# lzhangbj/deep_video_interpolation_extrapolation

Hardware: AMD Instinct MI355X
Metric: train frames/s (256x512 len-3 clips) (higher is better)
Workload: dtype bf16; 1 GPU; InterNet int_5_len_3 train step 256x512 bf16; per_gpu_batch=8, global_batch=8, parallelism=dp1, step=eager, executor side-stream lanes

## Files before the change

deep_video_interpolation_extrapolation_amd/csrc/ew.hip:

```cpp
#include <stdlib.h>

#include "common.h"

namespace dvie {

struct Lerp {
  int i0, i1;
  float l0, l1;
};
__device__ __forceinline__ Lerp lerp_src(int dst, int in_size, int out_size, int align) {
  float src;
  if (align) {
    const float scale = out_size > 1 ? (float)(in_size - 1) / (float)(out_size - 1) : 0.f;
    src = scale * (float)dst;
  } else {
    const float scale = (float)in_size / (float)out_size;
    src = scale * ((float)dst + 0.5f) - 0.5f;
  }
  if (src < 0.f) src = 0.f;
  Lerp r;
  r.i0 = (int)src;
  if (r.i0 > in_size - 1) r.i0 = in_size - 1;
  r.i1 = r.i0 + ((r.i0 < in_size - 1) ? 1 : 0);
  r.l1 = src - (float)r.i0;
// ... 333 lines not shown
#pragma unroll
      for (int k = 0; k < VW; ++k) v[k] += t[k];
    }
    if (p.beta) {
      VecN<T, VW>::load(yp, t);
#pragma unroll
      for (int k = 0; k < VW; ++k) v[k] += t[k];
    }
    if (p.act) {
#pragma unroll
      for (int k = 0; k < VW; ++k) v[k] = act_fwd(v[k], p.act, p.alpha);
    }
    if (p.dact) {
      VecN<T, VW>::load((const T*)p.z + pix * p.z_ld + c, t);
#pragma unroll
      for (int k = 0; k < VW; ++k) v[k] *= act_dz(t[k], p.dact, p.alpha);
    }
    VecN<T, VW>::store(yp, v);
  };
  finish(x, v0);
  if (two) finish(x + 1, v1);
}

template <int R>
__global__ __launch_bounds__(256) void ew_fuser_kernel(const dvie_ew_desc p, int cq) {
  const int e = blockIdx.x * 256 + threadIdx.x;
  const int sw = p.sw0, sh = p.sh0;
  if (e >= sw * cq) return;
  const int q = e / cq;
  const int c = (e - q * cq) * 8;
  const int row = blockIdx.y;
  const int n = row / p.h, y = row - (row / p.h) * p.h;
  const bf16_t* s = (const bf16_t*)p.src0;
  const long long ld = p.src_ld0;
  const Lerp ly = lerp_src(y, sh, p.h, 0);
  const long long r0 = ((long long)n * sh + ly.i0) * sw, r1 = ((long long)n * sh + ly.i1) * sw;
  const int qm = q > 0 ? q - 1 : 0, qp = q + 1 < sw ? q + 1 : sw - 1;
  float tm0[8], t00[8], tp0[8], tm1[8], t01[8], tp1[8];
  VecN<bf16_t, 8>::load(s + (r0 + qm) * ld + c, tm0);
  VecN<bf16_t, 8>::load(s + (r0 + q) * ld + c, t00);
  VecN<bf16_t, 8>::load(s + (r0 + qp) * ld + c, tp0);
  VecN<bf16_t, 8>::load(s + (r1 + qm) * ld + c, tm1);
  VecN<bf16_t, 8>::load(s + (r1 + q) * ld + c, t01);
  VecN<bf16_t, 8>::load(s + (r1 + qp) * ld + c, tp1);
#pragma unroll
  for (int r = 0; r < R; ++r) {
    const int x = R * q + r;
    if (x >= p.w) break;
    const Lerp lx = lerp_src(x, sw, p.w, 0);
    const bool lo = lx.i0 < q, hi = lx.i1 > q;
    float v[8];
#pragma unroll
    for (int k = 0; k < 8; ++k) {
      const float a = lo ? tm0[k] : t00[k], b = hi ? tp0[k] : t00[k];
      const float cc = lo ? tm1[k] : t01[k], d = hi ? tp1[k] : t01[k];
      v[k] = 0.f + (ly.l0 * (lx.l0 * a + lx.l1 * b) + ly.l1 * (lx.l0 * cc + lx.l1 * d));
    }
    const long long pix = (long long)row * p.w + x;
    bf16_t* yp = (bf16_t*)p.y + pix * p.y_ld + c;
    float t[8];
    if (p.res) {
      VecN<bf16_t, 8>::load((const bf16_t*)p.res + pix * p.res_ld + c, t);
#pragma unroll
      for (int k = 0; k < 8; ++k) v[k] += t[k];
    }
    if (p.beta) {
      VecN<bf16_t, 8>::load(yp, t);
#pragma unroll
      for (int k = 0; k < 8; ++k) v[k] += t[k];
    }
    if (p.act) {
#pragma unroll
      for (int k = 0; k < 8; ++k) v[k] = act_fwd(v[k], p.act, p.alpha);
    }
    if (p.dact) {
      VecN<bf16_t, 8>::load((const bf16_t*)p.z + pix * p.z_ld + c, t);
#pragma unroll
      for (int k = 0; k < 8; ++k) v[k] *= act_dz(t[k], p.dact, p.alpha);
    }
    VecN<bf16_t, 8>::store(yp, v);
  }
}

template <int R>
__global__ __launch_bounds__(256) void ew_upt22_kernel(const dvie_ew_desc p, int cq) {
  constexpr int NW = 3 * R;
  const int e = blockIdx.x * 256 + threadIdx.x;
  const int wp = (p.w + 1) >> 1, hp = (p.h + 1) >> 1;
  if (e >= wp * cq) return;
  const int xp = e / cq;
  const int c = (e - xp * cq) * 8;
  const int x = 2 * xp;
  const int rowp = blockIdx.y;
  const int n = rowp / hp, y = 2 * (rowp - (rowp / hp) * hp);
  const bool twox = x + 1 < p.w, twoy = y + 1 < p.h;
  const int sh = p.sh0, sw = p.sw0;
  const long long ld = p.src_ld0;
  const int Y0 = R * y - R / 2, X0 = R * x - R / 2;
  float wx0[NW], wx1[NW];
  unsigned xo[NW];
#pragma unroll
  for (int j = 0; j < NW; ++j) {
    const int X = X0 + j;
    const bool in = X >= 0 && X < sw;
    wx0[j] = in ? upt_weight(X, x, p.w, sw, 0) : 0.f;
    wx1[j] = (in && twox) ? upt_weight(X, x + 1, p.w, sw, 0) : 0.f;
    xo[j] = (unsigned)((in ? X : 0) * ld + c) * 2u;
  }
  const __amdgpu_buffer_rsrc_t rs = __builtin_amdgcn_make_buffer_rsrc((void*)p.src0, 0, 0x7FFFFFF0, 0x00020000);
  float acc[2][2][8];
#pragma unroll
  for (int a = 0; a < 2; ++a)
#pragma unroll
    for (int b = 0; b < 2; ++b)
#pragma unroll
      for (int k = 0; k < 8; ++k) acc[a][b][k] = 0.f;
#pragma unroll 1
  for (int i = 0; i < NW; ++i) {
    const int Y = Y0 + i;
    if (Y < 0 || Y >= sh) continue;
    const float wy0 = upt_weight(Y, y, p.h, sh, 0), wy1 = twoy ? upt_weight(Y, y + 1, p.h, sh, 0) : 0.f;
    if (wy0 == 0.f && wy1 == 0.f) continue;
    const unsigned rowo = (unsigned)(((long long)n * sh + Y) * sw * ld) * 2u;
    i32x4 raw[NW];
#pragma unroll
    for (int j = 0; j < NW; ++j) raw[j] = __builtin_bit_cast(i32x4, __builtin_amdgcn_raw_buffer_load_b128(rs, rowo + xo[j], 0, 0));
    float h0[8], h1[8];
#pragma unroll
    for (int k = 0; k < 8; ++k) h0[k] = h1[k] = 0.f;
#pragma unroll
    for (int j = 0; j < NW; ++j)
#pragma unroll
      for (int k = 0; k < 4; ++k) {
        const float lo = __uint_as_float(((uint32_t)raw[j][k]) << 16), hi = __uint_as_float(((uint32_t)raw[j][k]) & 0xffff0000u);
        h0[2 * k] += wx0[j] * lo;
        h0[2 * k + 1] += wx0[j] * hi;
        h1[2 * k] += wx1[j] * lo;
        h1[2 * k + 1] += wx1[j] * hi;
      }
#pragma unroll
    for (int k = 0; k < 8; ++k) {
      acc[0][0][k] += wy0 * h0[k];
      acc[0][1][k] += wy0 * h1[k];
      acc[1][0][k] += wy1 * h0[k];
      acc[1][1][k] += wy1 * h1[k];
    }
  }
  auto finish = [&](int yy, int xx, float* v) {
    const long long pix = ((long long)n * p.h + yy) * p.w + xx;
    bf16_t* yp = (bf16_t*)p.y + pix * p.y_ld + c;
    float t[8];
    if (p.res) {
      VecN<bf16_t, 8>::load((const bf16_t*)p.res + pix * p.res_ld + c, t);
#pragma unroll
      for (int k = 0; k < 8; ++k) v[k] += t[k];
    }
    if (p.beta) {
      VecN<bf16_t, 8>::load(yp, t);
#pragma unroll
      for (int k = 0; k < 8; ++k) v[k] += t[k];
    }
    if (p.act) {
#pragma unroll
      for (int k = 0; k < 8; ++k) v[k] = act_fwd(v[k], p.act, p.alpha);
    }
    if (p.dact) {
      VecN<bf16_t, 8>::load((const bf16_t*)p.z + pix * p.z_ld + c, t);
#pragma unroll
      for (int k = 0; k < 8; ++k) v[k] *= act_dz(t[k], p.dact, p.alpha);
    }
    VecN<bf16_t, 8>::store(yp, v);
  };
  finish(y, x, acc[0][0]);
  if (twox) finish(y, x + 1, acc[0][1]);
  if (twoy) {
    finish(y + 1, x, acc[1][0]);
    if (twox) finish(y + 1, x + 1, acc[1][1]);
  }
}

__global__ __launch_bounds__(256) void ew_nchw_kernel(const dvie_ew_desc p) {
  const int x = blockIdx.x * 256 + threadIdx.x;
  if (x >= p.w) return;
  const int row = blockIdx.y;
  const int n = row / p.h, y = row - (row / p.h) * p.h;
  const long long pix = (long long)row * p.w + x;
  const long long base = (long long)n * p.sn + (long long)y * p.sh + (long long)x * p.sw;
  if (p.c <= 32) {
    float v[32];
#pragma unroll
    for (int ch = 0; ch < 32; ++ch) {
      float t = 0.f;
      if (ch < p.c && ch < p.ext_c) {
        const bool second = p.src1 != nullptr && ch >= p.sh1;
        const float* e = second ? (const float*)p.src1 : p.ext;
        const int cc = second ? ch - p.sh1 : ch;
        t = e[base + (long long)cc * p.sc];
        if (p.mean) t = (t - p.mean[ch]) / p.std[ch];
      }
      v[ch] = t;
    }
#pragma unroll
    for (int c = 0; c < 32; c += 8)
      if (c < p.c) VecN<bf16_t, 8>::store((bf16_t*)p.y + pix * p.y_ld + c, v + c);
    return;
  }
  for (int c = 0; c < p.c; c += 8) {
    float v[8];
#pragma unroll
    for (int k = 0; k < 8; ++k) {
      const int ch = c + k;
      float t = 0.f;
      if (ch < p.ext_c) {
        const bool second = p.src1 != nullptr && ch >= p.sh1;
        const float* e = second ? (const float*)p.src1 : p.ext;
        const int cc = second ? ch - p.sh1 : ch;
        t = e[base + (long long)cc * p.sc];
        if (p.mean) t = (t - p.mean[ch]) / p.std[ch];
      }
      v[k] = t;
    }
    VecN<bf16_t, 8>::store((bf16_t*)p.y + pix * p.y_ld + c, v);
  }
}

template <typename T, int VW>
__global__ __launch_bounds__(256) void ew_labels_kernel(const dvie_ew_desc p, int cq) {
  const int e = blockIdx.x * 256 + threadIdx.x;
  if (e >= p.w * cq) return;
  const int x = e / cq;
  const int c = (e - x * cq) * VW;
  const int row = blockIdx.y;
  const int n = row / p.h, y = row - (row / p.h) * p.h;
  const uint8_t* lab = (const uint8_t*)p.ext;
  const int l = lab[(long long)n * p.sn + (long long)y * p.sh + (long long)x * p.sw];
  float v[VW];
#pragma unroll
  for (int k = 0; k < VW; ++k) v[k] = (c + k < p.ext_c && l == c + k) ? 1.f : 0.f;
  VecN<T, VW>::store((T*)p.y + ((long long)row * p.w + x) * p.y_ld + c, v);
}

}

using namespace dvie;

static bool fuse2_on() {
  const char* e = getenv("DVIE_EW_FUSE2");
  return !(e && *e == '0');
}

static int fuser_on() {
  const char* e = getenv("DVIE_EW_FUSER");
  return e && *e ? atoi(e) : 1;
}

extern "C" int dvie_ew(const dvie_ew_desc* d, void* stream) {
  DVIE_CHECK_ARG(d && d->c > 0 && d->c % 4 == 0, "ew: c=%d must be a multiple of 4", d ? d->c : -1);
  DVIE_CHECK_ARG(d->n > 0 && d->h > 0 && d->w > 0, "ew: empty shape");
  DVIE_CHECK_ARG(d->op == DVIE_EW_TONCHW || (d->y && d->y_ld % 4 == 0), "ew: y");
  if (d->op == DVIE_EW_POOL) DVIE_CHECK_ARG(d->sh0 == 2 * d->h && d->sw0 == 2 * d->w, "ew: pool shape");
  if (d->op == DVIE_EW_POOLT) DVIE_CHECK_ARG(d->h == 2 * d->sh0 && d->w == 2 * d->sw0, "ew: poolT shape");
  if (d->op == DVIE_EW_NCHW || d->op == DVIE_EW_TONCHW || d->op == DVIE_EW_MASK || d->op == DVIE_EW_LABELS)
    DVIE_CHECK_ARG(d->ext != nullptr, "ew: ext");
  if (d->op == DVIE_EW_LABELS)
    DVIE_CHECK_ARG(d->ext_c > 0 && d->ext_c <= 256 && !d->res && !d->beta && !d->act && !d->dact,
                   "ew: labels ext_c=%d (1..256), no epilogue operands", d->ext_c);
  if (d->dact) DVIE_CHECK_ARG(d->z != nullptr && d->z_ld % 4 == 0, "ew: z");
  if (d->op == DVIE_EW_IM2COL)
    DVIE_CHECK_ARG(d->ext_c > 0 && d->ext_c % 8 == 0 && d->src0 && d->src_ld0 >= d->ext_c &&
                       d->sh0 > 0 && d->sw0 > 0 && d->sh0 * d->sw0 * d->ext_c <= d->c,
                   "ew: im2col ext_c=%d c=%d taps=%dx%d", d->ext_c, d->c, d->sh0, d->sw0);
  DVIE_CHECK_ARG((long long)d->n * d->h < 65536 && (long long)d->w * d->c < (1LL << 30), "ew: grid too large");
  hipStream_t s = (hipStream_t)stream;
  auto al = [](const void* q, long long ld) { return !q || ((((uintptr_t)q) & 15) == 0 && ld % 8 == 0); };
  const bool v8 = d->dtype == DVIE_BF16 && d->c % 8 == 0 && al(d->y, d->y_ld) && al(d->src0, d->src_ld0) &&
                  al(d->src1, d->src_ld1) && al(d->src2, d->src_ld2) && al(d->res, d->res_ld) && al(d->z, d->z_ld);
  const int vw = v8 ? 8 : 4;
  const int cq = d->c / vw;
  const dim3 grid((unsigned)((d->w * cq + 255) / 256), (unsigned)(d->n * d->h));
  if (d->op == DVIE_EW_LABELS) {
    if (d->dtype == DVIE_BF16 && v8)
      DVIE_LAUNCH((ew_labels_kernel<bf16_t, 8>), grid, dim3(256), 0, s, *d, cq);
    else if (d->dtype == DVIE_BF16)
      DVIE_LAUNCH((ew_labels_kernel<bf16_t, 4>), grid, dim3(256), 0, s, *d, cq);
    else
      DVIE_LAUNCH((ew_labels_kernel<float, 4>), grid, dim3(256), 0, s, *d, cq);
    DVIE_RETURN_LAUNCH();
  }
  if (d->dtype == DVIE_BF16) {
    if (v8) {
      const bool up = d->sw0 <= d->w && d->sh0 <= d->h && (d->nsrc < 2 || (d->sw1 <= d->w && d->sh1 <= d->h)) &&
                      (d->nsrc < 3 || (d->sw2 <= d->w && d->sh2 <= d->h));
      if (d->op == DVIE_EW_NCHW && !d->res && !d->beta && !d->act && !d->dact) {
        const dim3 gn((unsigned)((d->w + 255) / 256), (unsigned)(d->n * d->h));
        DVIE_LAUNCH(ew_nchw_kernel, gn, dim3(256), 0, s, *d);
      } else if (d->op == DVIE_EW_FUSE && d->nsrc == 1 && !d->align && fuser_on() &&
                 ((d->h == 4 * d->sh0 && d->w == 4 * d->sw0) || (fuser_on() > 1 && d->h == 2 * d->sh0 && d->w == 2 * d->sw0))) {
        const dim3 gr((unsigned)((d->sw0 * cq + 255) / 256), (unsigned)(d->n * d->h));
        if (d->w == 4 * d->sw0)
          DVIE_LAUNCH((ew_fuser_kernel<4>), gr, dim3(256), 0, s, *d, cq);
        else
          DVIE_LAUNCH((ew_fuser_kernel<2>), gr, dim3(256), 0, s, *d, cq);
      } else if (d->op == DVIE_EW_FUSE && up && fuse2_on()) {
        const dim3 g2((unsigned)((((d->w + 1) / 2) * cq + 255) / 256), (unsigned)(d->n * d->h));
        DVIE_LAUNCH((ew_fuse2_kernel<bf16_t, 8>), g2, dim3(256), 0, s, *d, cq);
      } else if (d->op == DVIE_EW_FUSE)
        DVIE_LAUNCH((ew_kernel<bf16_t, 8, DVIE_EW_FUSE>), grid, dim3(256), 0, s, *d, cq);
      else if (d->op == DVIE_EW_UPT && !d->align &&
               (unsigned long long)d->n * d->sh0 * d->sw0 * d->src_ld0 * 2ull < 0x7FFFFFF0ull &&
               ((d->sh0 == 2 * d->h && d->sw0 == 2 * d->w) || (d->sh0 == 4 * d->h && d->sw0 == 4 * d->w))) {
        const dim3 g4((unsigned)((((d->w + 1) / 2) * cq + 255) / 256), (unsigned)(d->n * ((d->h + 1) / 2)));
        if (d->sh0 == 4 * d->h)
          DVIE_LAUNCH((ew_upt22_kernel<4>), g4, dim3(256), 0, s, *d, cq);
        else
          DVIE_LAUNCH((ew_upt22_kernel<2>), g4, dim3(256), 0, s, *d, cq);
      } else if (d->op == DVIE_EW_UPT)
        DVIE_LAUNCH((ew_kernel<bf16_t, 8, DVIE_EW_UPT>), grid, dim3(256), 0, s, *d, cq);
      else
        DVIE_LAUNCH((ew_kernel<bf16_t, 8, -2>), grid, dim3(256), 0, s, *d, cq);
    } else {
      DVIE_LAUNCH((ew_kernel<bf16_t, 4, -1>), grid, dim3(256), 0, s, *d, cq);
    }
  } else {
    DVIE_LAUNCH((ew_kernel<float, 4, -1>), grid, dim3(256), 0, s, *d, cq);
  }
  DVIE_RETURN_LAUNCH();
}
```

deep_video_interpolation_extrapolation_amd/engine.py:

```python
import ctypes
import os
from typing import NamedTuple, Optional

import torch

from . import _lib as L

PADC = 8
PROFILE = None
DEBUG_NAN = bool(os.environ.get("DVIE_DEBUG_NAN"))
def _wgrad_lane():
    return os.environ.get("DVIE_WGRAD_LANE", "1") != "0"


OP_HOOK = None


def pack_blocks(d):
    n = L.load().dvie_pack_blocks(ctypes.byref(d))
    assert n > 0, "dvie_pack_blocks: empty pack descriptor"
    return n


def _reduce_meta(name, r):
# ... 559 lines not shown
    size = [rup(max(int(b), 1), ARENA_ALIGN) for b, _, _ in items]
    order = sorted(range(len(items)), key=lambda i: (-size[i], items[i][1], i))
    offsets = [0] * len(items)
    placed = []
    arena = 0
    for i in order:
        _, f, l = items[i]
        busy = sorted((offsets[j], offsets[j] + size[j]) for j in placed if items[j][1] <= l and f <= items[j][2])
        off = 0
        for lo, hi in busy:
            if off + size[i] <= lo:
                break
            off = max(off, hi)
        offsets[i] = off
        placed.append(i)
        arena = max(arena, off + size[i])
    if arena > sum(size):
        offsets, arena = [], 0
        for sz in size:
            offsets.append(arena)
            arena += sz
    return offsets, arena


def arena_layout(g, nf):
    life = forward_lifetimes(g, nf)
    n_sites = max([b for _, b in life.values()] + [0])
    bufs = [b for b in g.buffers if not b.external]
    items = []
    for b in bufs:
        nbytes = nf * b.H * b.W * b.C * elem_size(b.dtype or g.dtype)
        items.append((nbytes,) + life.get(id(b), (0, n_sites)))
    offsets, arena = assign_offsets(items)
    return {id(b): o for b, o in zip(bufs, offsets)}, arena, sum(it[0] for it in items)


class Plan:

    def __init__(self, g, nf, nb, device, backward, alias=False):
        assert not (alias and backward), "alias=True is for forward-only plans (a backward reads every activation)"
        self.g, self.nf, self.nb, self.device, self.alias = g, nf, nb, device, alias
        self.dtype = g.dtype
        self.dt = dv_dtype(g.dtype)
        self.es = elem_size(g.dtype)
        self.vec = 16 // self.es
        self.backward_enabled = backward
        self.keep = []
        self.busy = False
        self.generation = 0
        self.static_weights = False
        self._pack_srcs, self._pack_sig, self._pack_descs = [], None, []
        self.arena, self.arena_bytes, self.unaliased_bytes = None, None, 0
        self.l1_out = self.bn_partial = None
        self.bn_splits = 1
        self._seg_bwd, self._seg_inner = {}, set()
        self.fwd = []
        self.bwd = []
        self.fwd_arr = self.bwd_arr = None
        self.fwd_off = self.n_bwd = 0
        self._l1_fwd = []
        self._l1_bwd = []
        self._cos_fwd = []
        self.cos_ws_blocks = 0
        self.ext_in = {}
        self.ext_out = {}
        self.ext_mask = {}
        self.ext_nchw_out = {}
        self.ext_head = {}
        self.ext_head_grad = {}
        self.keep_grad = None
        self.ext_grad = {}
        self._grad_slots = []
        self.ext_ograd = {}
        self.wg_first = {}
        self._uses_left = {}
        self.completions = []
        self._multi = []
        self._i2c = None
        self.ws = None
        self.ws_floats = 1
        self.zbits = {}
        self._zbits_level = int(os.environ.get("DVIE_ZBITS", "1") or 0)
        self._zbits_on = self._zbits_level > 0
        self._fwd_conv = {}
        self._zb = {}
        self._alloc()
        self._build_pack()
        self._build_forward()
        if backward:
            self._build_backward()
        assert all(o.lane == 0 for o in self.fwd), "forward ops run on the caller's stream"
        self._finalize()

    def _alloc(self):
        g = self.g
        offsets, self.arena_bytes, self.unaliased_bytes = arena_layout(g, self.nf) if self.alias else ({}, None, 0)
        if self.alias:
            self.arena = torch.empty(max(self.arena_bytes, ARENA_ALIGN), dtype=torch.uint8, device=self.device)
            self.keep.append(self.arena)
        for b in g.buffers:
            dt = b.dtype or self.dtype
            b.dt = dt
            if b.external:
                b.t = None
            elif self.alias:
                nbytes = self.nf * b.H * b.W * b.C * elem_size(dt)
                o = offsets[id(b)]
                b.t = self.arena[o:o + nbytes].view(dt).view(self.nf, b.H, b.W, b.C)
            else:
                b.t = torch.empty((self.nf, b.H, b.W, b.C), dtype=dt, device=self.device)
                self.unaliased_bytes += b.t.numel() * b.t.element_size()
        if self.backward_enabled:
            for op in g.ops:
                if op.out is None:
                    continue
                need = False
                if isinstance(op, InputOp):
                    need = op.requires_grad
                elif isinstance(op, (ConvOp, ConvTOp)):
                    need = op.layer.trainable or any(r.buf.needs_grad for r in op.inputs())
                elif isinstance(op, BNOp):
                    need = op.trainable or op.x.buf.needs_grad
                elif isinstance(op, FuseOp) and op.detach:
                    need = False
                else:
                    need = any(r.buf.needs_grad for r in op.inputs())
                op.out.buf.needs_grad = op.out.buf.needs_grad or need
            self._seg_bwd = self._segenc_bwd_chains()
            self._seg_inner = {id(op.out.buf) for ch in self._seg_bwd.values() for op in ch[:2]}
            for b in g.buffers:
                if b.needs_grad and id(b) not in self._seg_inner:
                    b.g = torch.zeros((self.nb, b.H, b.W, b.C), dtype=self.dtype, device=self.device)
            for b in g.buffers:
                b.expected, b.pending = {}, {}
                b.n_flushed = 0
                b.done = b.dact_done = False
            for op in g.ops:
                if isinstance(op, FuseOp) and op.detach:
                    continue
                for r in op.inputs():
                    if r.buf.needs_grad:
                        r.buf.expected[r.key()] = r.buf.expected.get(r.key(), 0) + 1
            for b in g.buffers:
                keys = sorted(b.expected)
                for (a0, ac), (b0, _) in zip(keys, keys[1:]):
                    assert a0 + ac <= b0, f"{b}: consumers read overlapping regions {keys}"
        self.l1_out = torch.zeros(max(1, g.n_l1), dtype=torch.float32, device=self.device)
        self.keep.append(self.l1_out)
        doubles = 8
        for op in g.ops:
            if isinstance(op, BNOp):
                d = L.BnDesc()
                d.c = op.x.c
                for n in (self.nf, self.nb):
                    d.rows = n * op.x.H * op.x.W
                    self.bn_splits = max(self.bn_splits, L.load().dvie_bn_partial_splits(ctypes.byref(d)))
                    doubles = max(doubles, L.load().dvie_bn_partial_doubles(ctypes.byref(d)))
                op.stats = torch.zeros((8, op.x.c), dtype=torch.float32, device=self.device)
                self.keep.append(op.stats)
        self.bn_partial = torch.zeros(doubles, dtype=torch.float64, device=self.device)
        self.keep.append(self.bn_partial)

    def ptr(self, region, n0=0, grad=False):
        b = region.buf
        t = b.g if grad else b.t
        es = elem_size(t.dtype)
# ... 345 lines not shown
        cb = sum(b.c for b in op.bs)
        moved = {"l2norm": 4 * op.c, "softmax": 3 * J, "wnorm": 4 * J, "pool": 2 * op.c,
                 "corr": op.c + J + cb, "gather": out.c + J + cb}[op.kind]

        def contrib(region, build):
            if region.buf.needs_grad:
                def emit(epi):
                    o = build(epi._asdict())
                    o.meta = dict(cls="attn_bwd", name=f"{op.kind}:{region.buf.name}", flops=0.0,
                                  bytes=float(self.es * npx * moved))
                    return [o]
                self._contrib(region, emit)

        if op.kind == "l2norm":
            contrib(a, lambda e: self.attn_desc(L.ATTN_L2NORM_BWD, nb, hw, op.c, gout, gld, self.ptr(a, grad=True),
                                                ld_a, self.ptr(out), self.ptr(a), self._same_ld(out, a), **e))
        elif op.kind == "softmax":
            contrib(a, lambda e: self.attn_desc(L.ATTN_SOFTMAX_BWD, nb, hw, op.c, gout, gld, self.ptr(a, grad=True),
                                                ld_a, self.ptr(out), None, out.buf.C, op.wh, op.ww, op.nhalf, **e))
        elif op.kind == "wnorm":
            contrib(a, lambda e: self.attn_desc(L.ATTN_WNORM_BWD, nb, hw, op.c, gout, gld, self.ptr(a, grad=True),
                                                ld_a, self.ptr(out), self.ptr(a), self._same_ld(out, a), op.wh,
                                                op.ww, op.nhalf, **e))
        elif op.kind == "pool":
            contrib(a, lambda e: self.attn_desc(L.ATTN_POOL_T, nb, hw, op.c, gout, gld, self.ptr(a, grad=True), ld_a,
                                                wh=op.wh, ww=op.ww, **e))
        elif op.kind == "corr":
            bs = op.bs
            bp = [self.ptr(b) for b in bs] + [None]
            contrib(a, lambda e: self.attn_desc(L.ATTN_GATHER, nb, hw, op.c, gout, gld, self.ptr(a, grad=True), ld_a,
                                                bp[0], bp[1], bs[0].buf.C, op.wh, op.ww, op.nhalf, 0, **e))
            for m, b in enumerate(bs):
                contrib(b, lambda e, m=m, b=b: self.attn_desc(
                    L.ATTN_GATHER_T, nb, hw, op.c, gout, gld, self.ptr(b, grad=True), b.buf.C, self.ptr(a), None,
                    ld_a, op.wh, op.ww, op.nhalf, m, **e))
        elif op.kind == "gather":
            fs = op.bs
            maps = [None] * op.nhalf
            for m, f in enumerate(fs):
                maps[op.half0 + m] = self.ptr(f)
            assert op.nhalf <= 2
            maps += [None]
            contrib(a, lambda e: self.attn_desc(L.ATTN_CORR, nb, hw, out.c, gout, gld, self.ptr(a, grad=True), ld_a,
                                                maps[0], maps[1], fs[0].buf.C, op.wh, op.ww, op.nhalf, **e))
            for m, f in enumerate(fs):
                contrib(f, lambda e, m=m, f=f: self.attn_desc(
                    L.ATTN_GATHER_T, nb, hw, out.c, self.ptr(a), ld_a, self.ptr(f, grad=True), f.buf.C, gout, None,
                    gld, op.wh, op.ww, op.nhalf, op.half0 + m, **e))
        else:
            raise TypeError(op.kind)

    @staticmethod
    def _same_ld(r0, r1):
        assert r0.buf.C == r1.buf.C, f"attn backward: {r0.buf} and {r1.buf} need one pixel stride"
        return r0.buf.C

    def _bn_common(self, d, op, n):
        x, m = op.x, op.m
        d.x, d.x_ld = self.ptr(x), x.buf.C
        d.rows, d.c = n * x.H * x.W, x.c
        d.splits = L.load().dvie_bn_partial_splits(ctypes.byref(d))
        d.partial, d.stats = self.bn_partial.data_ptr(), op.stats.data_ptr()
        d.gamma = m.weight.data_ptr() if m.weight is not None else None
        d.beta = m.bias.data_ptr() if m.bias is not None else None
        d.running_mean = m.running_mean.data_ptr() if m.running_mean is not None else None
        d.running_var = m.running_var.data_ptr() if m.running_var is not None else None
        assert m.num_features == x.c or rup(m.num_features, PADC) == x.c
        assert m.num_features == x.c, "BatchNorm channel count must be a multiple of 8"
        d.training = int(self.g.bn_training)
        d.act, d.alpha, d.eps = op.act, 0.2, m.eps
        d.x_f32 = int(x.buf.dt == torch.float32 and self.dtype != torch.float32)
        d.momentum = m.momentum if m.momentum is not None else 0.0
        d.dtype = self.dt

    def _contrib(self, region, emitter, ident=None):
        b = region.buf
        key = region.key()
        assert key in b.expected, (b, key)
        pend = b.pending.setdefault(key, [])
        pend.append((emitter, ident))
        if len(pend) == b.expected[key]:
            self._flush(b, key)

    def _flush(self, b, key):
        c0, c = key
        region = Region(b, c0, c)
        pending = b.pending.pop(key)
        kernels = [e for e, i in pending if e is not None]
        idents = [i for e, i in pending if e is None]
        prod = b.producers
        fuse_dact = False
        if len(prod) == 1 and prod[0].act != L.ACT_NONE and prod[0].out.buf is b:
            o0, oc = prod[0].out.c0, prod[0].out.c
            fuse_dact = (all(o0 <= k0 and k0 + kc <= o0 + oc for k0, kc in b.expected) and
                         sum(kc for _, kc in b.expected) == oc)
        b.dact_done = fuse_dact
        dact = prod[0].act if fuse_dact else 0
        z = self.ptr(region) if fuse_dact else None
        if fuse_dact:
            assert b.dt == self.dtype
        seq = []
        k = 0
        for em in kernels:
            r = idents[k] if k < len(idents) else None
            k += 1 if r is not None else 0
            seq.append((em, r))
        rest = idents[k:]
        gptr, gld = self.ptr(region, grad=True), b.C

        def copy_em(a):
            return lambda epi: [self.ew_desc(L.EW_COPY, self.nb, b.H, b.W, c, gptr, gld, [(a[0], a[1], b.H, b.W)],
                                             **epi._asdict())]

        while rest:
            a = rest.pop(0)
            seq.append((copy_em(a), rest.pop(0) if rest else None))
        for i, (em, r) in enumerate(seq):
            epi = Epilogue(beta=0 if i == 0 else 1, res=r[0] if r else None, res_ld=r[1] if r else 0)
            if i == len(seq) - 1:
                epi = epi._replace(dact=dact, z=z, z_ld=b.C)
            n_placed = len(self.bwd)
            ops = em(epi)
            if fuse_dact and i == len(seq) - 1:
                self._zbits_region(b, region, prod[0], ops, self.bwd[n_placed:])
            self.bwd.extend(ops)
        b.n_flushed += 1
        b.done = b.n_flushed == len(b.expected)

    def _zbits_region(self, b, region, prod, ops, placed):
        if not self._zbits_on or self.dtype != torch.bfloat16 or prod.act not in (L.ACT_LRELU, L.ACT_RELU):
            return
        st = self._zb.setdefault(id(b), dict(buf=b, prod=prod, users=[], regions=set(), ok=True, t=None))
        fo = self._fwd_conv.get(id(prod))
        if not ops and any(o.kind == L.OP_HEAD3_BWD and o.u.head3.dact for o in placed):
            st["regions"].add(region.key())
            return
        dact_of = {L.OP_CONV: lambda o: o.u.conv.dact, L.OP_EW: lambda o: o.u.ew.dact, L.OP_ATTN: lambda o: o.u.attn.dact}
        carriers = [o for o in ops if dact_of.get(o.kind, lambda o: 1)(o)]
        if (fo is None or b.C % 8 or region.c0 % 8 or prod.out.c0 % 8 or not carriers
                or any(o.kind != L.OP_CONV for o in carriers)):
            st["ok"] = False
            return
        if st["t"] is None:
            st["t"] = torch.empty(self.nf * b.H * b.W * b.C // 8, dtype=torch.uint8, device=self.device)
        for o in carriers:
            d = o.u.conv
            d.zbits, d.zbits_ld = st["t"].data_ptr() + region.c0 // 8, b.C // 8
            st["users"].append((o, region))
            st["regions"].add(region.key())
            if not L.load().dvie_conv_zbits(ctypes.byref(d)):
                st["ok"] = False

    def _zbits_settle(self):
        for st in self._zb.values():
            b, prod = st["buf"], st["prod"]
            ok = st["ok"] and st["t"] is not None and len(st["regions"]) == len(b.expected)
            if ok:
                d = self._fwd_conv[id(prod)].u.conv
                d.zbits, d.zbits_ld = st["t"].data_ptr() + prod.out.c0 // 8, b.C // 8
                ok = 0 < L.load().dvie_conv_zbits(ctypes.byref(d)) <= self._zbits_level
                if not ok:
                    d.zbits, d.zbits_ld = None, 0
            if not ok:
                for o, _ in st["users"]:
                    o.u.conv.zbits, o.u.conv.zbits_ld = None, 0
                continue
            self.zbits[b.name] = st["t"]
            self.keep.append(st["t"])
            for o, r in st["users"]:
                d = o.u.conv
                o.meta["bytes"] -= float(d.n * d.oh * d.ow * d.cout) * (self.es - 0.125)
            fo = self._fwd_conv[id(prod)]
            fo.meta["bytes"] += float(self.nf * b.H * b.W * prod.out.c) / 8
        self._zb = {}

    def _ensure_dact(self, op):
        b = op.out.buf
        if op.act == L.ACT_NONE or b.dact_done:
# ... 102 lines not shown
        if not x.buf.needs_grad:
            return
        xg = self.ptr(x, grad=True)

        def em(epi):
            assert epi.res is None and epi.dact == 0, "head backward has no fused epilogue"
            o = self._op(L.OP_HEAD_BWD)
            d = o.u.head
            d.gx, d.gx_ld = xg, x.buf.C
            d.n, d.h, d.w, d.c, d.pool, d.dtype, d.beta = self.nb, x.H, x.W, x.c, op.pool, self.dt, epi.beta
            self.ext_head_grad[op.key] = len(self.bwd)
            return [o]

        self._contrib(x, em)

    def _l1feat_backward(self, op, gout, gld):
        a = op.a
        if not a.buf.needs_grad:
            return
        numel = (self.nf // 2) * a.H * a.W * a.c
        ap, bp, ld = self.ptr(a, 0), self.ptr(a, self.nf // 2), a.buf.C
        gp = self.ptr(a, grad=True)
        scale = op.weight / numel

        def em(epi):
            o = self.ew_desc(L.EW_L1SIGN, self.nb, a.H, a.W, a.c, gp, ld, [(ap, ld, a.H, a.W), (bp, ld, a.H, a.W)],
                             scale=scale, **epi._asdict())
            o.l1_seed = scale
            return [o]

        self._contrib(a, em)

    def _input_backward(self, op, gout, gld):
        if not op.requires_grad:
            return
        out = op.out
        o = self.ew_desc(L.EW_TONCHW, self.nb, out.H, out.W, out.c, 0, 0, [(gout, gld, out.H, out.W)])
        o.u.ew.ext_c = op.ext_c
        if op.normalize:
            o.u.ew.std = op.std_t.data_ptr()
        self.ext_grad.setdefault(op.key, []).append((len(self.bwd), op))
        self.bwd.append(o)

    def _bn_backward(self, op, gout, gld):
        x = op.x
        assert len(x.buf.consumers) == 1, "BatchNorm input must have no other reader"
        if not x.buf.needs_grad:
            return
        xg = self.ptr(x, grad=True)

        def em(epi):
            assert epi.res is None and epi.dact == 0, "BatchNorm backward has no fused epilogue"
            o = self._op(L.OP_BN_BWD)
            d = o.u.bn
            self._bn_common(d, op, self.nb)
            d.g, d.g_ld = gout, gld
            d.dx, d.dx_ld, d.beta_dx = xg, x.buf.C, epi.beta
            if op.trainable:
                self._grad_slots.append((len(self.bwd), op.m, "bn", op.m not in self.wg_first))
                self.wg_first[op.m] = True
            return [o]

        self._contrib(x, em)

    def _fuse_backward(self, op, gout, gld):
        if op.detach:
            return
        out = op.out

        def resize_t(s):
            sp = self.ptr(s, grad=True)

            def em(epi):
                o = self.ew_desc(L.EW_UPT, self.nb, s.H, s.W, s.c, sp, s.buf.C, [(gout, gld, out.H, out.W)],
                                 **epi._asdict())
                o.u.ew.align = int(op.align)
                return [o]
            return em

        for s in op.srcs:
            if not s.buf.needs_grad:
                continue
            if (s.H, s.W) == (out.H, out.W):
                self._contrib(s, None, ident=(gout, gld))
            else:
                self._contrib(s, resize_t(s))

    def _mask_backward(self, op, gout, gld):
        src, out = op.src, op.out
        if not src.buf.needs_grad:
            return
        sp = self.ptr(src, grad=True)

        def em(epi):
            o = self.ew_desc(L.EW_MASK, self.nb, src.H, src.W, src.c, sp, src.buf.C, [(gout, gld, out.H, out.W)],
                             **epi._asdict())
            o.u.ew.ext_c = int(op.inverse)
            self.ext_mask.setdefault(op.key, []).append(("bwd", len(self.bwd), op))
            return [o]

        self._contrib(src, em)

    def _pool_backward(self, op, gout, gld):
        x, out = op.x, op.out
        if not x.buf.needs_grad:
            return
        xp = self.ptr(x, grad=True)
        self._contrib(x, lambda epi: [self.ew_desc(L.EW_POOLT, self.nb, x.H, x.W, x.c, xp, x.buf.C,
                                                   [(gout, gld, out.H, out.W)], **epi._asdict())])

    def _head3_fusable(self, op, gld):
        lay, x, out = op.layer, op.x, op.out
        mode = os.environ.get("DVIE_HEAD3_FUSED", "1")
        if self.dtype != torch.bfloat16 or mode == "0" or (mode == "1" and lay.cout_p != 8):
            return False
        if os.environ.get("DVIE_IM2COL_DGRAD", "0") == "1":
            return False
        if not (lay.trainable and x.buf.needs_grad and op.res is None and lay.kh == 3 and lay.kw == 3
                and lay.stride == 1 and lay.pad == 1 and lay.dil == 1 and lay.cout_p in (8, 24)
                and x.c % 64 == 0 and (out.H, out.W) == (x.H, x.W)):
            return False
        if x.buf.expected.get(x.key(), 0) != 1 or lay.cmap_t is not None and lay.cin != x.c:
            return False
        npx = self.nb * x.H * x.W
        return npx * max(x.buf.C, gld) * 2 < 0xFFFFFF00

    def _emit_head3(self, op, gout, gld, phase, xg, dact):
        lay, x = op.layer, op.x
        ph, wt, kpad = phase
        splits = max(1, 256 // (x.c // 64))
        slabs = torch.empty(splits * lay.cout_p * 9 * x.c, dtype=torch.float32, device=self.device)
        self.keep.append(slabs)
        o = self._op(L.OP_HEAD3_BWD)
        d = o.u.head3
        d.g, d.h, d.wd, d.dh, d.ws = gout, self.ptr(x), wt.data_ptr(), xg, slabs.data_ptr()
        d.g_ld, d.h_ld, d.dh_ld = gld, x.buf.C, x.buf.C
        d.n, d.hgt, d.wid, d.c = self.nb, x.H, x.W, x.c
        d.cout, d.kpad, d.dy0, d.dx0 = lay.cout_p, kpad, ph["dy0"], ph["dx0"]
        d.splits, d.dact, d.alpha = splits, dact, 0.2
        npix = self.nb * x.H * x.W
        o.meta = dict(cls="conv_dgrad", name=lay.name + "+wgrad",
                      flops=2.0 * npix * lay.cout * lay.cin * 9 * 2,
                      bytes=float(self.es * (2 * npix * x.c + npix * lay.cout) + 4 * slabs.numel()))
        self.bwd.append(o)
        csplits = self._colsum_op(gout, gld, npix, lay.cout_p) if lay.has_bias else 0
        self._reduce_op(lay, "weight", splits, 9 * x.c, x.c, own=slabs)
        if lay.has_bias:
            self._reduce_op(lay, "bias", csplits)
        self._close_layer(lay)

    def _conv_backward(self, op, gout, gld):
        lay, x, out = op.layer, op.x, op.out
        nb = self.nb
        head3 = self._head3_fusable(op, gld)
        if lay.trainable and not head3:
            self._emit_wgrad(op, gout, gld)
        if op.res is not None and op.res.buf.needs_grad:
            self._contrib(op.res, None, ident=(gout, gld))
        if not x.buf.needs_grad:
            return
        phases = self._dgrad_weights(lay, x.H, x.W)
        xg = self.ptr(x, grad=True)

        def em(epi):
            if head3:
                if epi.beta == 0 and epi.res is None and epi.dact in (L.ACT_NONE, L.ACT_LRELU) and \
                        (epi.z is None or epi.z == self.ptr(x)) and len(phases) == 1:
                    self._emit_head3(op, gout, gld, phases[0], xg, epi.dact)
                    return []
                self._emit_wgrad(op, gout, gld)
            extra = (epi.res is not None) + (epi.z is not None) + epi.beta
            if self._im2col_dgrad(lay, x, phases):
                return self._im2col_dgrad_ops(lay, x, xg, out, gout, gld, phases[0], epi)
            if self._ph4_eligible(lay, x):
                wt, kpad = self._dgrad_weights_ph4(lay)
                taps = dict(th=2, tw=2, dy0=0, dx0=0, ddy=1, ddx=1)
                o = self.conv_desc(gout, gld, nb, out.H, out.W, lay.cout_p, wt.data_ptr(), kpad, 4 * x.c, out.H,
                                   out.W, 1, 1, taps, xg, x.buf.C, x.H, x.W, osy=2, osx=2, **epi._asdict())
                o.u.conv.phc = x.c
                npx = nb * x.H * x.W
                o.meta = dict(cls="conv_dgrad", name=lay.name,
                              flops=2.0 * nb * out.H * out.W * lay.cin * lay.cout * 9,
                              bytes=float(self.es * (nb * out.H * out.W * lay.cout + npx * lay.cin * (1 + extra)
                                                     + lay.cout * lay.cin * 9)))
                return [o]
            ops = []
            for ph, wt, kpad in phases:
                o = self.conv_desc(
                    gout, gld, nb, out.H, out.W, lay.cout_p, wt.data_ptr(), kpad, x.c, ph["oh"], ph["ow"], 1, 1,
                    ph, xg, x.buf.C, x.H, x.W, osy=lay.stride, osx=lay.stride, ory=ph["ry"], orx=ph["rx"],
                    **epi._asdict())
                npx = nb * ph["oh"] * ph["ow"]
                frac = npx / float(nb * x.H * x.W)
                o.meta = dict(cls="conv_dgrad",
                              name=lay.name + (f" [phase {ph['ry']}{ph['rx']}]" if len(phases) > 1 else ""),
                              flops=2.0 * npx * lay.cin * lay.cout * ph["th"] * ph["tw"],
                              bytes=float(self.es * (frac * nb * out.H * out.W * lay.cout + npx * lay.cin * (1 + extra)
                                                     + lay.cout * lay.cin * ph["th"] * ph["tw"])))
                ops.append(o)
            return ops

        self._contrib(x, em)

    def _wgrad_s2_eligible(self, lay, x, out):
        mode = os.environ.get("DVIE_WGRAD_S2", "1")
        if mode == "1" and x.c < 256:
            return False
        return (self.dtype == torch.bfloat16 and mode != "0" and lay.stride == 2
                and lay.kh == 3 and lay.kw == 3 and lay.pad == 1 and lay.dil == 1 and not lay.transposed
                and x.H % 2 == 0 and x.W % 2 == 0 and out.H == x.H // 2 and out.W == x.W // 2 and out.W % 64 == 0
                and x.c % 8 == 0 and x.buf.C % 8 == 0)

    def _wgrad_op(self, g, g_ld, x, x_ld, oh, ow, cout, ih, iw, c, stride, taps, bias=False, ws_taps=0, tmap=0,
                  need_hint=False):
        o = self._op(L.OP_WGRAD)
        d = o.u.wgrad
        d.g, d.x, d.ws = g, x, 0
        d.g_ld, d.x_ld = g_ld, x_ld
        d.n, d.oh, d.ow, d.cout = self.nb, oh, ow, cout
        d.ih, d.iw, d.c, d.sy, d.sx = ih, iw, c, stride, stride
        d.th, d.tw, d.dy0, d.dx0, d.ddy, d.ddx = (taps[k] for k in ("th", "tw", "dy0", "dx0", "ddy", "ddx"))
        d.tmap, d.ws_taps, d.dtype = tmap, ws_taps, self.dt
        lib = L.load()
        hint = lib.dvie_wgrad_splits_hint(ctypes.byref(d))
        assert hint > 0 or not need_hint, "the halo weight-gradient kernel refused a launch lowered for it"
        ntap = taps["th"] * taps["tw"]
        tiles = rup(cout, 64) // 64 * (rup(c, 64) // 64)
        bkp = 64 if self.dtype == torch.bfloat16 else 32
        d.splits = hint if hint > 0 else max(1, min(max(1, self.nb * oh * ow // (bkp * 4)),
                                                    1024 // max(1, tiles * ntap)))
        slabs = lib.dvie_wgrad_slabs(ctypes.byref(d))
        wfl = slabs * cout * (ws_taps or ntap) * c
        bslabs = 0
        if bias:
            d.bws = 1
            bslabs = lib.dvie_wgrad_bias_slabs(ctypes.byref(d))
            d.bws = None
            o.bws_off = wfl
        self.ws_floats = max(self.ws_floats, wfl + bslabs * cout)
        return o, slabs, bslabs

# ... 513 lines not shown
```

Baseline: 264.1 frames/s.

## Add patch-based bilinear upsample-fuse kernel and software-pipelined upsample-transpose kernel

Adds a fuse kernel in which each thread loads a 3x3 neighbourhood of source pixels once and writes all RxR upsampled outputs from registers. Previously a thread was launched per output row and re-read the same source pixels. Adds a double-buffered variant of the upsample-transpose (UPT) backward kernel that issues the buffer loads for the next row before reducing the current one, to hide memory latency. Both are on by default via DVIE_EW_PATCH, and the patch path also enables the 2x fuse case, which previously needed fuser>1. Also adds an opt-in, default-off gradient aliasing path that shares an identity gradient buffer instead of copying it, and extends ident tuples to carry the source region.

```diff
diff --git a/deep_video_interpolation_extrapolation_amd/csrc/ew.hip b/deep_video_interpolation_extrapolation_amd/csrc/ew.hip
--- a/deep_video_interpolation_extrapolation_amd/csrc/ew.hip
+++ b/deep_video_interpolation_extrapolation_amd/csrc/ew.hip
@@ -439,6 +439,98 @@
   }
 }
 
+__device__ __forceinline__ void ew_finish8(const dvie_ew_desc& p, long long pix, int c, float* v) {
+  bf16_t* yp = (bf16_t*)p.y + pix * p.y_ld + c;
+  float t[8];
+  if (p.res) {
+    VecN<bf16_t, 8>::load((const bf16_t*)p.res + pix * p.res_ld + c, t);
+#pragma unroll
+    for (int k = 0; k < 8; ++k) v[k] += t[k];
+  }
+  if (p.beta) {
+    VecN<bf16_t, 8>::load(yp, t);
+#pragma unroll
+    for (int k = 0; k < 8; ++k) v[k] += t[k];
+  }
+  if (p.act) {
+#pragma unroll
+    for (int k = 0; k < 8; ++k) v[k] = act_fwd(v[k], p.act, p.alpha);
+  }
+  if (p.dact) {
+    VecN<bf16_t, 8>::load((const bf16_t*)p.z + pix * p.z_ld + c, t);
+#pragma unroll
+    for (int k = 0; k < 8; ++k) v[k] *= act_dz(t[k], p.dact, p.alpha);
+  }
+  VecN<bf16_t, 8>::store(yp, v);
+}
+
+__device__ __forceinline__ void unpack8(const i32x4 r, float* v) {
+#pragma unroll
+  for (int k = 0; k < 4; ++k) {
+    v[2 * k] = __uint_as_float(((uint32_t)r[k]) << 16);
+    v[2 * k + 1] = __uint_as_float(((uint32_t)r[k]) & 0xffff0000u);
+  }
+}
+
+__device__ __forceinline__ i32x4 sel4(bool s, const i32x4 a, const i32x4 b) { return s ? a : b; }
+
+__device__ __forceinline__ void lerp8(float* v, const Lerp ly, const Lerp lx, const i32x4 ra, const i32x4 rb,
+                                      const i32x4 rc, const i32x4 rd) {
+  float a[8], b[8], cc[8], d[8];
+  unpack8(ra, a);
+  unpack8(rb, b);
+  unpack8(rc, cc);
+  unpack8(rd, d);
+#pragma unroll
+  for (int k = 0; k < 8; ++k) v[k] += ly.l0 * (lx.l0 * a[k] + lx.l1 * b[k]) + ly.l1 * (lx.l0 * cc[k] + lx.l1 * d[k]);
+}
+
+template <int R>
+__global__ __launch_bounds__(256) void ew_fuser_kernel_patch(const dvie_ew_desc p, int cq) {
+  const int e = blockIdx.x * 256 + threadIdx.x;
+  const int sw = p.sw0, sh = p.sh0;
+  if (e >= sw * cq) return;
+  const int q = e / cq;
+  const int c = (e - q * cq) * 8;
+  const int srow = blockIdx.y;
+  const int n = srow / sh, pp = srow - (srow / sh) * sh;
+  const bf16_t* s = (const bf16_t*)p.src0 + c;
+  const long long ld = p.src_ld0;
+  const int rr[3] = {pp > 0 ? pp - 1 : 0, pp, pp + 1 < sh ? pp + 1 : sh - 1};
+  const int qq[3] = {q > 0 ? q - 1 : 0, q, q + 1 < sw ? q + 1 : sw - 1};
+  i32x4 t[3][3];
+#pragma unroll
+  for (int i = 0; i < 3; ++i)
+#pragma unroll
+    for (int j = 0; j < 3; ++j) t[i][j] = *(const i32x4*)(s + (((long long)n * sh + rr[i]) * sw + qq[j]) * ld);
+  Lerp lxs[R];
+#pragma unroll
+  for (int r = 0; r < R; ++r) lxs[r] = lerp_src(R * q + r, sw, p.w, 0);
+#pragma unroll
+  for (int ry = 0; ry < R; ++ry) {
+    const int y = R * pp + ry;
+    const Lerp ly = lerp_src(y, sh, p.h, 0);
+    const bool ylo = ly.i0 < pp, yhi = ly.i1 > pp;
+    i32x4 top[3], bot[3];
+#pragma unroll
+    for (int j = 0; j < 3; ++j) {
+      top[j] = sel4(ylo, t[0][j], t[1][j]);
+      bot[j] = sel4(yhi, t[2][j], t[1][j]);
+    }
+#pragma unroll
+    for (int rx = 0; rx < R; ++rx) {
+      const Lerp lx = lxs[rx];
+      const bool lo = lx.i0 < q, hi = lx.i1 > q;
+      float v[8];
+#pragma unroll
+      for (int k = 0; k < 8; ++k) v[k] = 0.f;
+      lerp8(v, ly, lx, sel4(lo, top[0], top[1]), sel4(hi, top[2], top[1]), sel4(lo, bot[0], bot[1]),
+            sel4(hi, bot[2], bot[1]));
+      ew_finish8(p, ((long long)n * p.h + y) * p.w + R * q + rx, c, v);
+    }
+  }
+}
+
 template <int R>
 __global__ __launch_bounds__(256) void ew_upt22_kernel(const dvie_ew_desc p, int cq) {
   constexpr int NW = 3 * R;
@@ -536,6 +628,87 @@
   }
 }
 
+template <int R>
+__global__ __launch_bounds__(256) void ew_upt22_kernel_pipe(const dvie_ew_desc p, int cq) {
+  constexpr int NW = 3 * R;
+  const int e = blockIdx.x * 256 + threadIdx.x;
+  const int wp = (p.w + 1) >> 1, hp = (p.h + 1) >> 1;
+  if (e >= wp * cq) return;
+  const int xp = e / cq;
+  const int c = (e - xp * cq) * 8;
+  const int x = 2 * xp;
+  const int rowp = blockIdx.y;
+  const int n = rowp / hp, y = 2 * (rowp - (rowp / hp) * hp);
+  const bool twox = x + 1 < p.w, twoy = y + 1 < p.h;
+  const int sh = p.sh0, sw = p.sw0;
+  const long long ld = p.src_ld0;
+  const int Y0 = R * y - R / 2, X0 = R * x - R / 2;
+  float wx0[NW], wx1[NW];
+  unsigned xo[NW];
+#pragma unroll
+  for (int j = 0; j < NW; ++j) {
+    const int X = X0 + j;
+    const bool in = X >= 0 && X < sw;
+    wx0[j] = in ? upt_weight(X, x, p.w, sw, 0) : 0.f;
+    wx1[j] = (in && twox) ? upt_weight(X, x + 1, p.w, sw, 0) : 0.f;
+    xo[j] = (unsigned)((in ? X : 0) * ld + c) * 2u;
+  }
+  const __amdgpu_buffer_rsrc_t rs = __builtin_amdgcn_make_buffer_rsrc((void*)p.src0, 0, 0x7FFFFFF0, 0x00020000);
+  float acc[2][2][8];
+#pragma unroll
+  for (int a = 0; a < 2; ++a)
+#pragma unroll
+    for (int b = 0; b < 2; ++b)
+#pragma unroll
+      for (int k = 0; k < 8; ++k) acc[a][b][k] = 0.f;
+  const int ilo = Y0 < 0 ? -Y0 : 0, ihi = sh - Y0 < NW ? sh - Y0 : NW;
+  auto fetch = [&](i32x4* raw, int i) {
+    const unsigned rowo = (unsigned)(((long long)n * sh + Y0 + i) * sw * ld) * 2u;
+#pragma unroll
+    for (int j = 0; j < NW; ++j) raw[j] = __builtin_bit_cast(i32x4, __builtin_amdgcn_raw_buffer_load_b128(rs, rowo + xo[j], 0, 0));
+  };
+  auto reduce = [&](const i32x4* raw, int i) {
+    const int Y = Y0 + i;
+    const float wy0 = upt_weight(Y, y, p.h, sh, 0), wy1 = twoy ? upt_weight(Y, y + 1, p.h, sh, 0) : 0.f;
+    if (wy0 == 0.f && wy1 == 0.f) return;
+    float h0[8], h1[8];
+#pragma unroll
+    for (int k = 0; k < 8; ++k) h0[k] = h1[k] = 0.f;
+#pragma unroll
+    for (int j = 0; j < NW; ++j)
+#pragma unroll
+      for (int k = 0; k < 4; ++k) {
+        const float lo = __uint_as_float(((uint32_t)raw[j][k]) << 16), hi = __uint_as_float(((uint32_t)raw[j][k]) & 0xffff0000u);
+        h0[2 * k] += wx0[j] * lo;
+        h0[2 * k + 1] += wx0[j] * hi;
+        h1[2 * k] += wx1[j] * lo;
+        h1[2 * k + 1] += wx1[j] * hi;
+      }
+#pragma unroll
+    for (int k = 0; k < 8; ++k) {
+      acc[0][0][k] += wy0 * h0[k];
+      acc[0][1][k] += wy0 * h1[k];
+      acc[1][0][k] += wy1 * h0[k];
+      acc[1][1][k] += wy1 * h1[k];
+    }
+  };
+  i32x4 ra[NW], rb[NW];
+  fetch(ra, ilo);
+#pragma unroll 1
+  for (int i = ilo; i < ihi; i += 2) {
+    fetch(rb, i + 1 < ihi ? i + 1 : ihi - 1);
+    reduce(ra, i);
+    fetch(ra, i + 2 < ihi ? i + 2 : ihi - 1);
+    if (i + 1 < ihi) reduce(rb, i + 1);
+  }
+  ew_finish8(p, ((long long)n * p.h + y) * p.w + x, c, acc[0][0]);
+  if (twox) ew_finish8(p, ((long long)n * p.h + y) * p.w + x + 1, c, acc[0][1]);
+  if (twoy) {
+    ew_finish8(p, ((long long)n * p.h + y + 1) * p.w + x, c, acc[1][0]);
+    if (twox) ew_finish8(p, ((long long)n * p.h + y + 1) * p.w + x + 1, c, acc[1][1]);
+  }
+}
+
 __global__ __launch_bounds__(256) void ew_nchw_kernel(const dvie_ew_desc p) {
   const int x = blockIdx.x * 256 + threadIdx.x;
   if (x >= p.w) return;
@@ -609,6 +782,11 @@
 static int fuser_on() {
   const char* e = getenv("DVIE_EW_FUSER");
   return e && *e ? atoi(e) : 1;
+}
+
+static bool patch_on() {
+  const char* e = getenv("DVIE_EW_PATCH");
+  return !(e && *e == '0');
 }
 
 extern "C" int dvie_ew(const dvie_ew_desc* d, void* stream) {
@@ -651,6 +829,13 @@
       if (d->op == DVIE_EW_NCHW && !d->res && !d->beta && !d->act && !d->dact) {
         const dim3 gn((unsigned)((d->w + 255) / 256), (unsigned)(d->n * d->h));
         DVIE_LAUNCH(ew_nchw_kernel, gn, dim3(256), 0, s, *d);
+      } else if (d->op == DVIE_EW_FUSE && d->nsrc == 1 && !d->align && fuser_on() && patch_on() &&
+                 ((d->h == 4 * d->sh0 && d->w == 4 * d->sw0) || (d->h == 2 * d->sh0 && d->w == 2 * d->sw0))) {
+        const dim3 gp((unsigned)((d->sw0 * cq + 255) / 256), (unsigned)(d->n * d->sh0));
+        if (d->w == 4 * d->sw0)
+          DVIE_LAUNCH((ew_fuser_kernel_patch<4>), gp, dim3(256), 0, s, *d, cq);
+        else
+          DVIE_LAUNCH((ew_fuser_kernel_patch<2>), gp, dim3(256), 0, s, *d, cq);
       } else if (d->op == DVIE_EW_FUSE && d->nsrc == 1 && !d->align && fuser_on() &&
                  ((d->h == 4 * d->sh0 && d->w == 4 * d->sw0) || (fuser_on() > 1 && d->h == 2 * d->sh0 && d->w == 2 * d->sw0))) {
         const dim3 gr((unsigned)((d->sw0 * cq + 255) / 256), (unsigned)(d->n * d->h));
@@ -667,7 +852,11 @@
                (unsigned long long)d->n * d->sh0 * d->sw0 * d->src_ld0 * 2ull < 0x7FFFFFF0ull &&
                ((d->sh0 == 2 * d->h && d->sw0 == 2 * d->w) || (d->sh0 == 4 * d->h && d->sw0 == 4 * d->w))) {
         const dim3 g4((unsigned)((((d->w + 1) / 2) * cq + 255) / 256), (unsigned)(d->n * ((d->h + 1) / 2)));
-        if (d->sh0 == 4 * d->h)
+        if (patch_on() && d->sh0 == 4 * d->h)
+          DVIE_LAUNCH((ew_upt22_kernel_pipe<4>), g4, dim3(256), 0, s, *d, cq);
+        else if (patch_on())
+          DVIE_LAUNCH((ew_upt22_kernel_pipe<2>), g4, dim3(256), 0, s, *d, cq);
+        else if (d->sh0 == 4 * d->h)
           DVIE_LAUNCH((ew_upt22_kernel<4>), g4, dim3(256), 0, s, *d, cq);
         else
           DVIE_LAUNCH((ew_upt22_kernel<2>), g4, dim3(256), 0, s, *d, cq);
diff --git a/deep_video_interpolation_extrapolation_amd/engine.py b/deep_video_interpolation_extrapolation_amd/engine.py
--- a/deep_video_interpolation_extrapolation_amd/engine.py
+++ b/deep_video_interpolation_extrapolation_amd/engine.py
@@ -665,6 +665,7 @@
         self.zbits = {}
         self._zbits_level = int(os.environ.get("DVIE_ZBITS", "1") or 0)
         self._zbits_on = self._zbits_level > 0
+        self._grad_alias = os.environ.get("DVIE_GRAD_ALIAS", "0") == "1"
         self._fwd_conv = {}
         self._zb = {}
         self._alloc()
@@ -1176,6 +1177,19 @@
         if len(pend) == b.expected[key]:
             self._flush(b, key)
 
+    def _alias_identity(self, b, key, kernels, idents):
+        if not self._grad_alias or kernels or len(idents) != 1 or len(b.expected) != 1 or key != (0, b.C):
+            return False
+        if any(p.act != L.ACT_NONE for p in b.producers):
+            return False
+        src = idents[0][2]
+        sb = src.buf
+        if (sb is b or sb.g is None or b.g is None or src.key() != (0, sb.C) or sb.g.shape != b.g.shape
+                or sb.g.dtype != b.g.dtype):
+            return False
+        b.g = sb.g
+        return True
+
     def _flush(self, b, key):
         c0, c = key
         region = Region(b, c0, c)
@@ -1188,6 +1202,11 @@
             o0, oc = prod[0].out.c0, prod[0].out.c
             fuse_dact = (all(o0 <= k0 and k0 + kc <= o0 + oc for k0, kc in b.expected) and
                          sum(kc for _, kc in b.expected) == oc)
+        if self._alias_identity(b, key, kernels, idents):
+            b.dact_done = True
+            b.n_flushed += 1
+            b.done = True
+            return
         b.dact_done = fuse_dact
         dact = prod[0].act if fuse_dact else 0
         z = self.ptr(region) if fuse_dact else None
@@ -1456,7 +1475,7 @@
             if not s.buf.needs_grad:
                 continue
             if (s.H, s.W) == (out.H, out.W):
-                self._contrib(s, None, ident=(gout, gld))
+                self._contrib(s, None, ident=(gout, gld, out))
             else:
                 self._contrib(s, resize_t(s))
 
@@ -1530,7 +1549,7 @@
         if lay.trainable and not head3:
             self._emit_wgrad(op, gout, gld)
         if op.res is not None and op.res.buf.needs_grad:
-            self._contrib(op.res, None, ident=(gout, gld))
+            self._contrib(op.res, None, ident=(gout, gld, out))
         if not x.buf.needs_grad:
             return
         phases = self._dgrad_weights(lay, x.H, x.W)
```

Measured after the change: 264.6 frames/s, median of 6. Within noise of the previous version (+0.2%).
